# furio1999/EO_Diffusion

Hardware: AMD Instinct MI355X
Metric: denoising steps/sec (UNet fwd + DDPM update) at 256x256 bs=16 (higher is better)
Workload: dtype f32; 1 GPU; DDPM sampling step, 256x256x3, batch 16 per GPU, UNet arch A0 (base 128, mults [1,2,3,4], 1 res-block(s), attn_res []), Philox noise, x0-clipped update; global_batch=16, image_size=256, parallelism=batch-sharded x1, accumulate=fp32, precision_mode=fp32x3

## Files before the change

eo_diffusion_amd/_lib.py:

```python
import ctypes as C
import os

_HERE = os.path.dirname(os.path.abspath(__file__))
LIB_PATH = os.environ.get("EOD_LIBRARY") or os.path.join(_HERE, "lib", "libeodiff.so")

EOD_F32, EOD_F16 = 0, 1
ATTN_OUT_PRESPLIT, ATTN_IN_PRESPLIT, ATTN_EXACT_F32 = 1, 2, 4
(OP_CONV, OP_GEMM, OP_GN_PARTIAL, OP_GN_FINALIZE, OP_GN_APPLY, OP_SOFTMAX, OP_TEMB, OP_TO_NHWC, OP_TO_NCHW,
 OP_POOL, OP_ATTN, OP_TRANSPOSE, OP_ATTN_NAT, OP_DROPOUT, OP_ACT_BOUND, OP_BOUND_AFFINE) = range(1, 17)

vp, i32, i64, f32, f64 = C.c_void_p, C.c_int32, C.c_int64, C.c_float, C.c_double


class ConvDesc(C.Structure):
    _fields_ = [("x", vp), ("x2", vp), ("w", vp), ("bias", vp), ("cbias", vp), ("res", vp), ("y", vp),
                ("cbias_stride", i64), ("dtype", i32), ("N", i32), ("H", i32), ("W", i32), ("C0", i32), ("C1", i32),
                ("Cout", i32), ("ksize", i32), ("stride", i32), ("pad", i32), ("upsample", i32), ("pad_tl", i32),
                ("Ho", i32), ("Wo", i32), ("out_nchw_f32", i32), ("alpha", f32), ("stats", vp), ("stats_slots", i32),
                ("gn_silu", i32), ("gn_scale_shift", vp), ("workspace", vp), ("workspace_bytes", i64),
                ("w_tapmajor", i32), ("w_split", i32), ("w_scale", vp), ("a_bound", vp),
                ("skip_x", vp), ("skip_x2", vp), ("skip_w", vp), ("skip_C0", i32), ("skip_C1", i32), ("skip_bound", vp), ("x_presplit", i32), ("y_presplit_bound", vp)]


class GemmDesc(C.Structure):
# ... 67 lines not shown
    "eod_dropout": (i32, [vp, vp, i32, i64, f32, C.c_uint64, C.c_uint32, C.c_uint32, vp]),
    "eod_rowdot": (i32, [vp, vp, i32, i64, i64, i64, i64, i64, i64, i32, vp, vp]),
    "eod_scale_f32": (i32, [vp, i64, f32, vp]),
    "eod_attention_fwd_nat": (i32, [vp, vp, vp, i32, i32, i32, i32, i32, i32, i32, i32, i32, i32, vp, i32, vp]),
    "eod_weight_l1max": (i32, [vp, i32, i32, vp, vp, vp]),
    "eod_bound_affine": (i32, [vp, vp, vp, i32, vp]),
    "eod_attention_bwd": (i32, [vp, vp, vp, vp, vp, i32, i32, i32, i32, i32, i32, i32, i32, i32, i32, vp]),
    "eod_gemm_tn": (i32, [vp, i64, vp, i64, vp, i64, i32, i32, i32, i32, f32, i32, i32, i64, i64, i64, i64, i64, i64, vp]),
    "eod_softmax_bwd_rows": (i32, [vp, i64, vp, i64, vp, i32, i64, i32, vp]),
    "eod_linear_bwd_small": (i32, [vp, i64, vp, vp, vp, vp, vp, i32, i32, i32, i32, f32, vp, vp, vp, vp, vp]),
    "eod_temb_pre1": (i32, [vp, vp, vp, vp, i32, i32, i32, vp, vp]),
    "eod_embedding_bwd": (i32, [vp, vp, i32, i32, i32, f32, vp, vp]),
    "eod_mse_loss": (i32, [vp, vp, i64, vp, vp, vp, i32, vp]),
    "eod_adamw_step": (i32, [vp, vp, vp, vp, i64, f64, f64, f64, f64, f64, i32, vp]),
    "eod_adamw_step_guarded": (i32, [vp, vp, vp, vp, i64, f64, f64, f64, f64, f64, i32, vp, vp, i32, vp]),
    "eod_ema_update": (i32, [vp, vp, i64, f64, vp]),
    "eod_pack_rows": (i32, [vp, i64, vp, vp, i64, i32, i32, i32, vp]),
    "eod_nchw_to_nhwc": (i32, [vp, i32, vp, i32, vp, i32, i32, i32, i32, i32, vp]),
    "eod_nhwc_to_nchw": (i32, [vp, i32, vp, i32, i32, i32, i32, vp]),
    "eod_gn_partial": (i32, [vp, i32, i32, i32, i32, vp, i32, i32, i32, vp]),
    "eod_gn_finalize": (i32, [vp, i32, i32, vp, i32, i32, i32, i64, i32, f32, vp, vp, vp, i64, vp, vp, vp, vp]),
    "eod_act_bound": (i32, [vp, i32, i32, i64, vp, i32, i32, vp, i32, i32, vp, i32, vp]),
    "eod_conv_stats_slots": (i32, [C.POINTER(ConvDesc)]),
    "eod_conv_gn_fusable": (i32, [C.POINTER(ConvDesc)]),
    "eod_conv_split_ok": (i32, [C.POINTER(ConvDesc)]),
    "eod_conv_skip_ok": (i32, [C.POINTER(ConvDesc)]),
    "eod_conv_up4_ok": (i32, [C.POINTER(ConvDesc)]),
    "eod_conv_up4_weights": (i32, [vp, vp, i32, i32, vp]),
    "eod_conv_up4_bwd_ok": (i32, [C.POINTER(ConvDesc)]),
    "eod_pack_conv_weight_split": (i32, [vp, vp, vp, i32, i32, i32, i32, vp]),
    "eod_pack_conv_weight_split_pair": (i32, [vp, vp, vp, vp, vp, i32, i32, i32, i32, i32, vp]),
    "eod_conv_workspace_size": (i64, [C.POINTER(ConvDesc)]),
    "eod_conv_kernel_name": (C.c_char_p, [C.POINTER(ConvDesc)]),
    "eod_gn_apply": (i32, [vp, i32, i32, i32, i32, vp, i32, i32, i32, vp, vp, vp]),
    "eod_attention_fwd": (i32, [C.POINTER(AttnDesc), vp]),
    "eod_softmax_rows": (i32, [vp, i64, vp, i64, i32, i64, i32, vp]),
    "eod_time_embed": (i32, [C.POINTER(TembDesc), vp]),
    "eod_timestep_embedding": (i32, [vp, vp, vp, i32, i32, vp]),
    "eod_q_sample": (i32, [vp, vp, vp, vp, vp, vp, i32, i64, i32, vp]),
    "eod_repaint_mix": (i32, [vp, vp, vp, vp, vp, vp, vp, vp, i32, i32, i64, i32, vp]),
    "eod_ddpm_step": (i32, [vp, vp, vp, vp, vp, vp, vp, vp, vp, i32, i64, i32, i32, vp]),
    "eod_ddim_step": (i32, [vp, vp, vp, f32, f32, f32, f32, f32, vp, vp, i64, vp]),
    "eod_cfg_combine": (i32, [vp, vp, f32, vp, i64, vp]),
    "eod_dpmpp_step": (i32, [vp, vp, vp, f32, f32, f32, f32, f32, f32, i32, vp, vp, i64, vp]),
    "eod_ddim_step_obs": (i32, [vp, vp, vp, f32, f32, f32, f32, f32, vp, vp, f32, C.POINTER(i32), i32, i32, i32, i32, i32, i32, i32, vp, vp, vp]),
    "eod_dpmpp_step_obs": (i32, [vp, vp, vp, f32, f32, f32, f32, f32, f32, i32, vp, vp, f32, C.POINTER(i32), i32, i32, i32, i32, i32, i32, i32,
                                 vp, vp, vp]),
    "eod_block_mean": (i32, [vp, C.POINTER(i32), vp, i32, i32, i32, i32, vp]),
    "eod_obs_project": (i32, [vp, vp, vp, f32, C.POINTER(i32), i32, i32, i32, i32, i32, i32, i32, vp, vp]),
    "eod_ddim_step_spec": (i32, [vp, vp, vp, f32, f32, f32, f32, f32, vp, vp, f32, C.POINTER(f32), C.POINTER(f32), i32, i32, i32, i32, i32, i32,
                                 i32, i32, vp, vp, vp]),
    "eod_dpmpp_step_spec": (i32, [vp, vp, vp, f32, f32, f32, f32, f32, f32, i32, vp, vp, f32, C.POINTER(f32), C.POINTER(f32), i32, i32, i32, i32,
                                  i32, i32, i32, i32, vp, vp, vp]),
    "eod_spec_project": (i32, [vp, vp, vp, f32, C.POINTER(f32), C.POINTER(f32), i32, i32, i32, i32, i32, i32, i32, i32, vp, vp]),
    "eod_spec_apply": (i32, [vp, C.POINTER(f32), i32, i32, vp, i32, i32, i32, i32, vp]),
    "eod_psf_residual": (i32, [vp, vp, vp, f32, C.POINTER(f32), i32, i32, C.POINTER(i32), i32, i32, i32, i32, i32, i32, i32, i32, vp, vp]),
    "eod_psf_apply": (i32, [vp, C.POINTER(f32), i32, i32, C.POINTER(i32), i32, vp, i32, i32, i32, i32, vp]),
    "eod_psf_update": (i32, [vp, vp, f32, C.POINTER(f32), i32, i32, C.POINTER(i32), i32, i32, i32, i32, i32, vp, vp]),
    "eod_psf_residual_mix": (i32, [vp, vp, vp, f32, C.POINTER(f32), i32, i32, C.POINTER(f32), i32, i32, i32, i32, i32, i32, i32, vp, vp]),
    "eod_psf_apply_mix": (i32, [vp, C.POINTER(f32), i32, i32, C.POINTER(f32), i32, vp, i32, i32, i32, i32, vp]),
    "eod_psf_update_mix": (i32, [vp, vp, f32, C.POINTER(f32), i32, i32, C.POINTER(f32), i32, i32, i32, i32, i32, vp, vp]),
    "eod_psf_residual_xy": (i32, [vp, vp, vp, f32, C.POINTER(f32), i32, C.POINTER(f32), i32, i32, C.POINTER(i32), C.POINTER(f32), i32, i32, i32, i32, i32,
                                  i32, i32, i32, vp, vp]),
    "eod_psf_apply_xy": (i32, [vp, C.POINTER(f32), i32, C.POINTER(f32), i32, i32, C.POINTER(i32), C.POINTER(f32), i32, vp, i32, i32, i32, i32, vp]),
    "eod_psf_update_xy": (i32, [vp, vp, f32, C.POINTER(f32), i32, C.POINTER(f32), i32, i32, C.POINTER(i32), C.POINTER(f32), i32, i32, i32, i32, i32,
                                vp, vp]),
# ... 22 lines not shown
    "eod_scene_stack_tile_active": (i32, [vp, vp, i32, i32, i32, i32, i32, vp, vp, i32, i32, vp]),
    "eod_scene_stack_keep_known": (i32, [vp, vp, vp, i32, vp, vp, i32, i32, i32, i32, i32, i32, i32, vp, vp]),
    "eod_scene_stats": (i32, [vp, vp, vp, i32, i64, vp]),
    "eod_program_run": (i32, [C.POINTER(Op), i32, vp]),
    "eod_timer_create": (vp, [i32, i32]),
    "eod_timer_destroy": (None, [vp]),
    "eod_timer_read": (i32, [vp, C.POINTER(f32)]),
    "eod_timer_set_mask": (i32, [vp, vp, i32]),
    "eod_program_run_timed": (i32, [C.POINTER(Op), i32, vp, vp]),
    "eod_resample2x": (i32, [vp, i32, i32, i32, i32, i32, i32, i32, vp, vp]),
}

_lib = None


class EodError(RuntimeError):
    pass


ABI_VERSION = 115
SPEC_GRID_BLOCKS = 4096


def lib():
    global _lib
    if _lib is not None:
        return _lib
    if not os.path.exists(LIB_PATH):
        raise EodError(
            f"libeodiff.so not found at {LIB_PATH}. Build it first (python -c 'import __graft_entry__ as g; g.build()' "
            "or make -C eo_diffusion_amd/csrc). There is no fallback path.")
    import torch
    L = C.CDLL(LIB_PATH)
    for name, (res, args) in SYMBOLS.items():
        fn = getattr(L, name)
        fn.restype, fn.argtypes = res, args
    if L.eod_version() != ABI_VERSION and os.environ.get("EOD_ABI_ANY", "0") != "1":
        raise EodError(f"ABI mismatch: {LIB_PATH} was built for revision {L.eod_version()} of include/eodiff.h, this binding mirrors {ABI_VERSION}")
    for kind, st in ((1, ConvDesc), (2, GemmDesc), (3, TembDesc), (4, SmallDesc), (5, Op), (6, AttnDesc)):
        if L.eod_struct_size(kind) != C.sizeof(st):
            raise EodError(f"ABI mismatch: struct kind {kind}: C {L.eod_struct_size(kind)} vs ctypes {C.sizeof(st)}")
    _lib = L
    return L


def check(rc, what=""):
    if rc != 0:
        msg = lib().eod_last_error()
        raise EodError(f"{what} failed (rc={rc}): {msg.decode() if msg else ''}")


def dtype_id(torch_dtype):
    import torch
    if torch_dtype == torch.float16:
        return EOD_F16
    if torch_dtype == torch.float32:
        return EOD_F32
    raise EodError(f"unsupported storage dtype {torch_dtype}")


def ptr(t):
    return 0 if t is None else t.data_ptr()
```

eo_diffusion_amd/csrc/igemm.hip:

```cpp
#include <type_traits>

#include "common.h"

struct IgemmP {
    const char* a0;
    const char* a1;
    const char* b;
    const float* bias;
    const float* cbias;
    const char* res;
    char* y;
    long long cbias_stride;
    int N, H, W, C0, C1, Cin, Cout, KS, stride, pad, ups, pad_tl, Ho, Wo, HoWo, Heff, Weff;
    int tw_log2, th;
    int tiles_pw, tiles_pi;
    long long lda, ldb, ldc, sa0, sa1, sb0, sb1, sc0, sc1;
    int nb1, bias_mode, c_f32;
    long long M;
    int Ncols, K, taps, KT, tiles_m, tiles_n, out_nchw;
    int kc0, kc1;
    int tapmajor_log2;
    int ldk;
    const float* gn_ss;
    int gn_silu;
// ... 133 lines not shown
            g.ty0 = ty * p.th;
            g.tx0 = (t - ty * p.tiles_pw) << p.tw_log2;
        } else {
            const long long m0 = (long long)tile_m * BM;
            g.n_first = (int)(m0 / p.HWd);
            g.rem_first = (int)(m0 - (long long)g.n_first * p.HWd);
        }
    } else {
        const int z = blockIdx.y;
        const int b0 = z / p.nb1, b1 = z - b0 * p.nb1;
        g.offA = b0 * p.sa0 + b1 * p.sa1;
        g.offB = b0 * p.sb0 + b1 * p.sb1;
        g.offC = b0 * p.sc0 + b1 * p.sc1;
    }
    return g;
}

#ifdef EOD_STAMP
__device__ unsigned long long g_eod_stamp[65536][16];
#define EOD_STAMP_AT(k)                                                                    \
    do {                                                                                   \
        if (threadIdx.x == 0 && blockIdx.x < 65536) {                                      \
            g_eod_stamp[blockIdx.x][2 * (k)] = __builtin_amdgcn_s_memrealtime();           \
            g_eod_stamp[blockIdx.x][2 * (k) + 1] = __builtin_amdgcn_s_memtime();           \
        }                                                                                  \
    } while (0)
extern "C" int eod_debug_read_stamps(unsigned long long* host, int n) {
    return (int)hipMemcpyFromSymbol(host, HIP_SYMBOL(g_eod_stamp), (size_t)n * 16 * sizeof(unsigned long long), 0, hipMemcpyDeviceToHost);
}
#else
#define EOD_STAMP_AT(k) do { } while (0)
#endif
#ifdef EOD_TSTAMP
__device__ unsigned long long g_eod_tstamp[2048][40];
extern "C" int eod_debug_read_tstamps(unsigned long long* host, int n) {
    return (int)hipMemcpyFromSymbol(host, HIP_SYMBOL(g_eod_tstamp), (size_t)n * 40 * sizeof(unsigned long long), 0, hipMemcpyDeviceToHost);
}
#define EOD_TSTAMP_AT(idx)                                                                                      \
    do {                                                                                                        \
        if (GN && wave == 1 && cc == 1 && k == 0) {                                                             \
            const unsigned long long ts_ = __builtin_amdgcn_s_memtime();                                        \
            if (lane == 0) reinterpret_cast<unsigned long long*>(sA + ABUF + PR * 128)[idx] = ts_;              \
        }                                                                                                       \
    } while (0)
#else
#define EOD_TSTAMP_AT(idx) do { } while (0)
#endif
__device__ __forceinline__ void map_tile(const IgemmP& p, int& tile_m, int& tile_n) {
    const int nwg = gridDim.x, bid = blockIdx.x;
    const int xcd = bid & 7, q = nwg >> 3, r = nwg & 7;
    const int swz = (xcd < r ? xcd * (q + 1) : r * (q + 1) + (xcd - r) * q) + (bid >> 3);
    tile_n = swz % p.tiles_n;
    tile_m = swz / p.tiles_n;
}

template <int MS> struct AccLayout {
    static constexpr int R = MS == 32 ? 16 : 4;
    typedef typename std::conditional<MS == 32, f32x16, f32x4>::type vec;
    static __device__ __forceinline__ int row(int r, int lane) { return MS == 32 ? (r & 3) + 8 * (r >> 2) + 4 * (lane >> 5) : 4 * (lane >> 4) + r; }
    static __device__ __forceinline__ int col(int lane) { return MS == 32 ? (lane & 31) : (lane & 15); }
};

template <typename T, bool CONV, int BM, int BN, int WAVES_M, int WAVES_N, bool OUTF32, int MS = 32>
__device__ __forceinline__ void igemm_epilogue(const IgemmP& p, const TileGeom& g,
                                               typename AccLayout<MS>::vec (&acc)[BM / WAVES_M / MS][BN / WAVES_N / MS], char* smem, int wave,
                                               int lane, int n0, const float* rowtab = nullptr, int rowtab_n = 0,
                                               const float* pre_bcol = nullptr) {
    constexpr int ES = sizeof(T);
    constexpr int WM = BM / WAVES_M, WN = BN / WAVES_N;
    constexpr int TM = WM / MS, TN = WN / MS, R = AccLayout<MS>::R;
    constexpr int EP_LD = WN + 4;
    const int wm = wave / WAVES_N, wn = wave % WAVES_N;
    const int lr = AccLayout<MS>::col(lane);
// ... 712 lines not shown
    } else {
        if (CONV ? p.splitk > 1 : p.c_f32 != 0)
            igemm_epilogue<T, CONV, BM, BN, WAVES_M, WAVES_N, true, MS>(pe, g, acc, smem, wave, lane, n0);
        else
            igemm_epilogue<T, CONV, BM, BN, WAVES_M, WAVES_N, false, MS>(pe, g, acc, smem, wave, lane, n0);
    }
}

template <int TN, int MS>
__device__ __forceinline__ void prefetch_bcol(const IgemmP& p, int ncols, int col0, int lane, int n_first, float (&out)[TN]) {
    const int lr = AccLayout<MS>::col(lane);
#pragma unroll
    for (int j = 0; j < TN; ++j) {
        const int col = col0 + j * MS + lr;
        const bool ok = col < ncols;
        float v = (ok && p.bias && p.bias_mode == 1) ? p.bias[col] : 0.0f;
        if (ok && p.cbias) v += p.cbias[(long long)n_first * p.cbias_stride + col];
        out[j] = v;
    }
}

template <typename T, int BN, int WAVES_M, int WAVES_N, bool UPS, bool GN, bool SPLIT = false, int MS = 32, bool SKIP = false, bool KSPLIT = false>
__global__ __launch_bounds__(64 * WAVES_M * WAVES_N, WAVES_N == 4 ? 1 : 2) void conv3x3_halo_kernel(const IgemmP p) {
    static_assert(!KSPLIT || (!UPS && BN == 128), "K slices: the 128-column 4-wave instances");
    static_assert(!SKIP || (MS == 16 && !UPS && WAVES_M == 2), "fused skip conv: 16x16x32 instances of the 8x16 tile");
    static_assert(!SPLIT || (sizeof(T) == 4 && MS == 16), "the split-fp16 product is a mode of fp32 storage, on 16x16x32 MFMAs");
    static_assert(MS == 32 || SPLIT || sizeof(T) == 2, "the 16x16x32 shape exists for the fp16 products only");
    constexpr bool XF = GN || SPLIT;
    constexpr bool DIRECT = SPLIT && MS == 16 && BN >= 64;
    constexpr int NW = WAVES_M * WAVES_N;
    constexpr int BM = WAVES_N == 4 ? 64 * WAVES_M : 32 * NW, TH = BM / 16, TW = 16;
    constexpr int PH = UPS ? TH / 2 + 2 : TH + 2, PW = UPS ? TW / 2 + 2 : TW + 2, PR = PH * PW;
    constexpr int PG = (PR + 7) / 8;
    constexpr int LAH = (PG + NW - 1) / NW;
    constexpr int ES = sizeof(T), EPC = 16 / ES, BKB = 128, BK = BKB / ES;
    constexpr int WM = BM / WAVES_M, WN = BN / WAVES_N, TM = WM / MS, TN = WN / MS;
    constexpr int GB = BN / 8, LB = GB / NW;
    constexpr int ABUF = PG * 1024, BSTAGE = BN * BKB, BSTAGES = 2;
    static_assert(GB % NW == 0 && LAH <= 6, "layout");

    extern __shared__ __attribute__((aligned(16))) char smem[];
    char* const sA = smem;
    char* const sB = smem + 2 * ABUF;
    char* const sS = sB + BSTAGES * BSTAGE;
    EOD_STAMP_AT(0);

    const int tid = threadIdx.x, lane = tid & 63;
    const int wave = __builtin_amdgcn_readfirstlane(tid >> 6);
    const int wm = wave / WAVES_N, wn = wave % WAVES_N;
    int tile_m, tile_n;
    map_tile(p, tile_m, tile_n);
    const int n0 = p.n_base + tile_n * BN;
    const TileGeom g = make_geom<true, BM>(p, tile_m);
    float pre_bcol[DIRECT ? 1 : TN];
    f32x4 pre_bq[DIRECT ? TN : 1];
    int pre_we[DIRECT ? TN : 1];
    if constexpr (DIRECT) {
        prefetch_bcol4<TN>(p, p.Ncols, n0 + wn * WN, lane, g.n_first, pre_bq);
        prefetch_wexp4<TN>(p, p.Ncols, n0 + wn * WN, p.w_row0, lane, pre_we);
    } else {
        prefetch_bcol<TN, MS>(p, p.Ncols, n0 + wn * WN, lane, g.n_first, pre_bcol);
    }
    float wsc1 = 1.0f;
    if constexpr (SPLIT) wsc1 = p.w_scale[1];
    AbScale asc = {EOD_SPLIT_ASCALE, 1.0f};
    const float silu_k = p.gn_silu ? -1.44269504088896341f : 0.0f, silu_c = p.gn_silu ? 0.0f : -__builtin_inff();
    if constexpr (SPLIT) {
        if (p.a_bound) asc = ab_scale_of(ab_wave_bound(p.a_bound, g.n_first));
        if constexpr (SKIP) {
            if (p.skip_bound) {
                const AbScale k = ab_scale_of(ab_wave_bound(p.skip_bound, g.n_first));
                if (k.s < asc.s) asc = k;
            }
        }
    }

    const int srow = lane >> 3, sslot = lane & 7;
    unsigned ppix[LAH];
    const int bchunk0 = sslot ^ ((4 * wave + (srow >> 1)) & 7);
    unsigned pck = 0;
    unsigned pvalid = 0;
#pragma unroll
    for (int i = 0; i < LAH; ++i) {
        const int prow = (wave + NW * i) * 8 + srow;
        const int px = prow - (prow / PW) * PW;
        pck |= (unsigned)(sslot ^ ((px >> 1) & 7)) << (3 * i);
    }
    auto set_tile_pieces = [&](const TileGeom& tg) {
#pragma unroll
        for (int i = 0; i < LAH; ++i) {
            const int prow = (wave + NW * i) * 8 + srow;
            const int py = prow / PW, px = prow - py * PW;
            const int hi = (UPS ? tg.ty0 / 2 : tg.ty0) - 1 + py, wi = (UPS ? tg.tx0 / 2 : tg.tx0) - 1 + px;
            const bool ok = (wave + NW * i) < PG && prow < PR && (unsigned)hi < (unsigned)p.H && (unsigned)wi < (unsigned)p.W;
            if (ok) pvalid |= 1u << i;
            ppix[i] = (unsigned)(hi * p.W + wi);
        }
    };
    set_tile_pieces(g);
    auto pchunk_of = [&](int i) { return (int)((pck >> (3 * i)) & 7u); };
    unsigned b_v[LB];
#pragma unroll
    for (int i = 0; i < LB; ++i) {
        const int row = (wave + NW * i) * 8 + srow;
        b_v[i] = (n0 + row < p.Ncols) ? (unsigned)(row * p.Cin * ES) + bchunk0 * 16 : EOD_OOB;
    }
    const __amdgpu_buffer_rsrc_t rsA0 = make_rsrc(p.a0 + (long long)g.n_first * p.H * p.W * p.C0 * ES);
    const __amdgpu_buffer_rsrc_t rsA1 = make_rsrc(p.a1 ? p.a1 + (long long)g.n_first * p.H * p.W * p.C1 * ES : p.a0);
    const __amdgpu_buffer_rsrc_t rsB = make_rsrc(p.b + (long long)n0 * p.Cin * ES);
    const int tapstride = p.Cout * p.Cin * ES;
    __amdgpu_buffer_rsrc_t rsS = rsB;
    if constexpr (GN)
        rsS = __builtin_amdgcn_make_buffer_rsrc(const_cast<float*>(p.gn_ss) + (long long)g.n_first * p.Cin * 2, 0, p.Cin * 8, 0x00020000);

    struct Chunk {
        int src, kin, cw;
        unsigned bk;
        bool ktail;
    };
    auto chunk_of = [&](int cc) {
        Chunk c;
        c.src = cc >= p.kc0 ? 1 : 0;
        const int ci = c.src ? cc - p.kc0 : cc;
        c.kin = ci * BK;
        c.cw = c.src ? p.C1 : p.C0;
        c.bk = (unsigned)(((c.src ? p.C0 : 0) + c.kin) * ES);
        c.ktail = c.kin + BK > c.cw;
        return c;
    };
    auto issue_patch_piece = [&](int i, const Chunk& c, char* abuf) {
        const int pc = pchunk_of(i);
        unsigned v = ((pvalid >> i) & 1u) ? ppix[i] * (unsigned)(c.cw * ES) + pc * 16 : EOD_OOB;
        if (__builtin_expect(c.ktail, 0)) v = (c.kin + pc * EPC < c.cw) ? v : EOD_OOB;
        if (c.src)
            blds16(rsA1, v, (unsigned)(c.kin * ES), abuf + (wave + NW * i) * 1024);
        else
            blds16(rsA0, v, (unsigned)(c.kin * ES), abuf + (wave + NW * i) * 1024);
    };
    auto issue_ss = [&](const Chunk& c, char* ssbuf) {
        const unsigned v = lane < 32 ? (unsigned)(lane * 16 + ((c.src ? p.C0 : 0) + c.kin) * 8) : EOD_OOB;
        __builtin_amdgcn_raw_ptr_buffer_load_lds(rsS, (lds_void*)ssbuf, 16, v, 0, 0, 0);
    };
    struct XfPre {
        i32x4 raw;
        f32x4 q[GN ? (ES == 2 ? 4 : 2) : 1];
    };
    auto xf_load = [&](int i, char* abuf, const char* ssbuf, XfPre& pre) {
        const int pc = pchunk_of(i);
        pre.raw = *reinterpret_cast<const i32x4*>(abuf + (wave + NW * i) * 1024 + lane * 16);
        if constexpr (GN) {
            const float* sp = reinterpret_cast<const float*>(ssbuf) + pc * EPC * 2;
#pragma unroll
            for (int k = 0; k < (ES == 2 ? 4 : 2); ++k) pre.q[k] = *reinterpret_cast<const f32x4*>(sp + 4 * k);
        }
    };
    auto xf_finish = [&](int i, const Chunk& c, char* abuf, const XfPre& pre) {
        const int pc = pchunk_of(i);
        const bool ok = ((pvalid >> i) & 1u) && (!c.ktail || (c.kin + pc * EPC < c.cw));
        char* ptr = abuf + (wave + NW * i) * 1024 + lane * 16;
        const i32x4 raw = pre.raw;
        i32x4 outv = raw;
        if constexpr (GN) {
            if constexpr (ES == 2) {
                const half8 h = __builtin_bit_cast(half8, raw);
                half8 o;
#pragma unroll
                for (int e = 0; e < 8; ++e) {
                    float v = (float)h[e] * pre.q[e >> 1][(e & 1) * 2] + pre.q[e >> 1][(e & 1) * 2 + 1];
                    v = v * __builtin_amdgcn_rcpf(1.0f + __builtin_amdgcn_exp2f(__builtin_fmaf(v, silu_k, silu_c)));
                    o[e] = (half_t)v;
                }
                outv = __builtin_bit_cast(i32x4, o);
            } else {
                const f32x4 f = __builtin_bit_cast(f32x4, raw);
                f32x4 o;
                const f32x4 q0 = pre.q[0], q1 = pre.q[GN && ES != 2 ? 1 : 0];
                const float sc[4] = {q0[0], q0[2], q1[0], q1[2]}, sh[4] = {q0[1], q0[3], q1[1], q1[3]};
#pragma unroll
                for (int e = 0; e < 4; ++e) {
                    float v = f[e] * sc[e] + sh[e];
                    if constexpr (SPLIT) {
                        v = v * __builtin_amdgcn_rcpf(1.0f + __builtin_amdgcn_exp2f(__builtin_fmaf(v, silu_k, silu_c)));
                    } else {
                        if (p.gn_silu) v = silu_f<SPLIT>(v);
                    }
                    o[e] = v;
                }
                outv = __builtin_bit_cast(i32x4, o);
            }
            if constexpr (!SPLIT) {
                if (!ok) outv = raw;
            }
        }
        if constexpr (SPLIT) {
            const float sl = (GN && !ok) ? 0.0f : asc.s;
            *reinterpret_cast<i32x4*>(ptr) = split_pair_exchange_scaled(__builtin_bit_cast(f32x4, outv), sl, (pc & 1) != 0);
        } else {
            if (ok) *reinterpret_cast<i32x4*>(ptr) = outv;
        }
    };
    auto transform_piece = [&](int i, const Chunk& c, char* abuf, const char* ssbuf) {
        XfPre pre;
        xf_load(i, abuf, ssbuf, pre);
        xf_finish(i, c, abuf, pre);
    };
    unsigned bve[LB];
    auto weight_offsets = [&](const Chunk& c, unsigned (&out)[LB]) {
        const bool kok = !c.ktail || (c.kin + (SPLIT ? (bchunk0 >> 1) * 8 : bchunk0 * EPC) < c.cw);
#pragma unroll
        for (int i = 0; i < LB; ++i) out[i] = kok ? b_v[i] : EOD_OOB;
    };
    auto issue_weights_at = [&](int tap, const Chunk& c, const unsigned (&off)[LB], char* bst) {
        const unsigned soff = (unsigned)(tap * tapstride) + c.bk;
#pragma unroll
        for (int i = 0; i < LB; ++i) blds16(rsB, off[i], soff, bst + (wave + NW * i) * 1024);
    };
    auto issue_weights = [&](int tap, const Chunk& c, char* bst) {
        unsigned off[LB];
        weight_offsets(c, off);
        issue_weights_at(tap, c, off, bst);
    };

    typename AccLayout<MS>::vec acc[TM][TN];
#pragma unroll
    for (int i = 0; i < TM; ++i)
#pragma unroll
        for (int j = 0; j < TN; ++j)
#pragma unroll
            for (int r = 0; r < AccLayout<MS>::R; ++r) acc[i][j][r] = 0.0f;

    const int lr = lane & (MS - 1), lh = MS == 32 ? lane >> 5 : lane >> 4;
    int prow0[TM], pyo[TM], pxo[TM];
#pragma unroll
    for (int i = 0; i < TM; ++i) {
        const int r = wm * WM + i * MS + lr;
        pyo[i] = r >> 4;
        pxo[i] = r & 15;
        prow0[i] = pyo[i] * PW + pxo[i];
    }
    const int bsw = (lr >> 1) & 7;
    int bcoff[4];
#pragma unroll
    for (int s = 0; s < 4; ++s) bcoff[s] = ((2 * s + lh) ^ bsw) * 16;
    const int b_rd = (wn * WN + lr) * BKB;
    int acur[2][3] = {{0, 0, 0}, {0, 0, 0}};
    auto aoff = [](int r) { return (UPS ? ((r + 1) >> 1) : r) * PW * BKB; };
    i32x4 aw[2][TM];
    auto a_load = [&](int v, int dx, int dy) {
#pragma unroll
        for (int r = 0; r < TM + 2; ++r)
            if (dy == 0 ? r < TM : r == TM - 1 + dy) aw[v][r % TM] = *reinterpret_cast<const i32x4*>(sA + acur[v][dx] + aoff(r));
    };
    constexpr bool EARLY = MS == 16 && WAVES_N == 4;
    auto tap_slot = [](int t) { return MS == 16 ? 3 * (t % 3) + t / 3 : t; };
    if constexpr (MS == 16) {
        constexpr int LROW = WM / 16;
        static_assert(LROW % 2 == 0, "the UPS row split needs an even first tile row per wave");
        const int c0 = SPLIT ? 2 * ((0x2130 >> (4 * lh)) & 3) : lh, c1 = SPLIT ? c0 + 1 : 4 + lh;
#pragma unroll
        for (int dx = 0; dx < 3; ++dx) {
            const int pxc = UPS ? ((lr + dx + 1) >> 1) : lr + dx;
            const int key = (pxc >> 1) & 7;
            const int rowb = ((UPS ? (wm * LROW) >> 1 : wm * LROW) * PW + pxc) * BKB;
            acur[0][dx] = rowb + ((c0 ^ key) << 4);
            acur[1][dx] = rowb + ((c1 ^ key) << 4);
        }
    }

    const int KC = p.kc0 + p.kc1;
    int kc_begin = 0, kc_end = KC;
    if constexpr (KSPLIT) {
        kc_begin = (int)blockIdx.y * p.splitk_per;
        kc_end = (int)blockIdx.y == p.splitk - 1 ? KC : kc_begin + p.splitk_per;
    }
    const int NSTEP = (kc_end - kc_begin) * 9;
    {
        const Chunk c0 = chunk_of(kc_begin);
#pragma unroll
        for (int i = 0; i < LAH; ++i)
            if ((wave + NW * i) < PG) issue_patch_piece(i, c0, sA);
        if constexpr (GN) {
            if (wave == 0) issue_ss(c0, sS);
        }
        issue_weights(0, c0, sB);
        if constexpr (XF) {
            asm volatile("s_waitcnt vmcnt(0)" ::: "memory");
            if constexpr (GN) __builtin_amdgcn_s_barrier();
#pragma unroll
            for (int i = 0; i < LAH; ++i)
                if ((wave + NW * i) < PG) transform_piece(i, c0, sA, sS);
            __builtin_amdgcn_s_waitcnt(0xc07f);
        }
    }
    EOD_STAMP_AT(1);
    int pp1 = 0;
    int step = 0;
    int qpar = 0;
    for (int once = 0; once < 1; ++once) {
    for (int cc = kc_begin; cc < kc_end; ++cc) {
        const Chunk cur = chunk_of(cc);
        const int cn = cc + 1 < kc_end ? cc + 1 : cc;
        const bool has_next = cn != cc;
        const Chunk nxt = chunk_of(cn);
        const char* abuf = sA + qpar * ABUF;
        char* abuf_next = sA + (qpar ^ 1) * ABUF;
        weight_offsets(cur, bve);
#pragma unroll
        for (int t = 0; t < 9; ++t, ++step) {
            EOD_TSTAMP_AT(4 * t + 0);
            if (pp1 == 0) asm volatile("s_waitcnt vmcnt(0)" ::: "memory");
            else if (pp1 == 1) asm volatile("s_waitcnt vmcnt(1)" ::: "memory");
            else asm volatile("s_waitcnt vmcnt(2)" ::: "memory");
            if constexpr (XF) __builtin_amdgcn_s_waitcnt(0xc07f);
            __builtin_amdgcn_s_barrier();
            EOD_TSTAMP_AT(4 * t + 1);
            if (step + 1 < NSTEP) {
                if (t < 8) issue_weights_at(tap_slot(t + 1), cur, bve, sB + ((step + 1) & 1) * BSTAGE);
                else issue_weights(0, nxt, sB + ((step + 1) & 1) * BSTAGE);
            }
            pp1 = 0;
            if (t < LAH && has_next && (wave + NW * t) < PG) {
                issue_patch_piece(t, nxt, abuf_next);
                pp1 = 1;
            }
            if constexpr (GN) {
                if (t == 0 && has_next && wave == 0) {
                    issue_ss(nxt, sS + (qpar ^ 1) * 1024);
                    ++pp1;
                }
            }
            EOD_TSTAMP_AT(4 * t + 2);
            const int dy = MS == 16 ? t % 3 : t / 3, dx = MS == 16 ? t / 3 : t % 3;
            const int ndy = (t + 1) % 3, ndx = (t + 1) / 3;
            const bool a_here = !EARLY || t == 0, a_early = EARLY && t < 8;
            const char* bst = sB + (step & 1) * BSTAGE;
            int arow[TM], asw[TM];
#pragma unroll
            for (int i = 0; i < TM; ++i) {
                const int pxc = UPS ? ((pxo[i] + dx + 1) >> 1) : pxo[i] + dx;
                const int prow = UPS ? ((pyo[i] + dy + 1) >> 1) * PW + pxc : prow0[i] + dy * PW + dx;
                arow[i] = prow * BKB;
                asw[i] = (pxc >> 1) & 7;
            }
            if constexpr (MS == 16 && SPLIT) {
                const int ch = 2 * ((0x2130 >> (4 * lh)) & 3);
                i32x4 bh[TN], bl[TN];
                if (a_here) a_load(1, dx, dy);
#pragma unroll
                for (int j = 0; j < TN; ++j) bh[j] = *reinterpret_cast<const i32x4*>(bst + b_rd + j * MS * BKB + ((ch ^ bsw) << 4));
                if (a_here) a_load(0, dx, dy);
#pragma unroll
                for (int i = 0; i < TM; ++i)
#pragma unroll
                    for (int j = 0; j < TN; ++j)
                        acc[i][j] = DIRECT ? __builtin_amdgcn_mfma_f32_16x16x32_f16(__builtin_bit_cast(half8, bh[j]), __builtin_bit_cast(half8, aw[1][(i + dy) % TM]), acc[i][j], 0, 0, 0)
                                           : __builtin_amdgcn_mfma_f32_16x16x32_f16(__builtin_bit_cast(half8, aw[1][(i + dy) % TM]), __builtin_bit_cast(half8, bh[j]), acc[i][j], 0, 0, 0);
#pragma unroll
                for (int j = 0; j < TN; ++j) bl[j] = *reinterpret_cast<const i32x4*>(bst + b_rd + j * MS * BKB + (((ch + 1) ^ bsw) << 4));
                if (a_early) a_load(1, ndx, ndy);
#pragma unroll
                for (int i = 0; i < TM; ++i)
#pragma unroll
// ... 20 lines not shown
#pragma unroll
                        for (int j = 0; j < TN; ++j)
                            acc[i][j] = __builtin_amdgcn_mfma_f32_16x16x32_f16(__builtin_bit_cast(half8, aw[s][(i + dy) % TM]), __builtin_bit_cast(half8, fb16[j]), acc[i][j], 0, 0, 0);
                    if (a_early) a_load(s, ndx, ndy);
                }
            } else {
            i32x4 fa[2][TM], fb[2][TN];
#pragma unroll
            for (int i = 0; i < TM; ++i)
                fa[0][i] = *reinterpret_cast<const i32x4*>(abuf + arow[i] + (((0 + lh) ^ asw[i]) << 4));
#pragma unroll
            for (int j = 0; j < TN; ++j) fb[0][j] = *reinterpret_cast<const i32x4*>(bst + b_rd + j * 32 * BKB + bcoff[0]);
            __builtin_amdgcn_sched_group_barrier(0x100, TM + TN, 0);
#pragma unroll
            for (int s = 0; s < 4; ++s) {
                const int cur = s & 1, nx = cur ^ 1;
                if (s < 3) {
#pragma unroll
                    for (int i = 0; i < TM; ++i)
                        fa[nx][i] = *reinterpret_cast<const i32x4*>(abuf + arow[i] + (((2 * (s + 1) + lh) ^ asw[i]) << 4));
#pragma unroll
                    for (int j = 0; j < TN; ++j)
                        fb[nx][j] = *reinterpret_cast<const i32x4*>(bst + b_rd + j * 32 * BKB + bcoff[s + 1]);
                    __builtin_amdgcn_sched_group_barrier(0x100, TM + TN, 0);
                }
#pragma unroll
                for (int i = 0; i < TM; ++i)
#pragma unroll
                    for (int j = 0; j < TN; ++j) Mma<T>::run(fa[cur][i], fb[cur][j], acc[i][j]);
                __builtin_amdgcn_sched_group_barrier(0x008, TM * TN * (sizeof(T) == 4 ? 4 : 1), 0);
            }
            }
            EOD_TSTAMP_AT(4 * t + 3);
            if constexpr (XF) {
                if (t >= 2 && t - 2 < LAH && has_next && (wave + NW * (t - 2)) < PG)
                    transform_piece(t - 2, nxt, abuf_next, sS + (qpar ^ 1) * 1024);
            }
        }
        EOD_TSTAMP_AT(36);
#ifdef EOD_TSTAMP
        if (GN && wave == 1 && cc == 1 && blockIdx.x < 2048) {
            __builtin_amdgcn_s_waitcnt(0xc07f);
            if (lane < 37) g_eod_tstamp[blockIdx.x][lane] = reinterpret_cast<const unsigned long long*>(sA + ABUF + PR * 128)[lane];
        }
#endif
        if constexpr (MS == 16) {
            const int flip = qpar ? -ABUF : ABUF;
#pragma unroll
            for (int dx = 0; dx < 3; ++dx) {
                acur[0][dx] += flip;
                acur[1][dx] += flip;
            }
        }
        qpar ^= 1;
    }
    if constexpr (SKIP) {
      if (!KSPLIT || (int)blockIdx.y == p.splitk - 1) {
        constexpr int LA = BM / 8 / NW;
        constexpr int STG_A = BM * BKB, STG = STG_A + BSTAGE;
        static_assert(2 * STG <= 2 * ABUF + BSTAGES * BSTAGE, "the skip phase reuses the operand ring");
        __builtin_amdgcn_s_waitcnt(0xc07f);
        __builtin_amdgcn_s_barrier();
        const int SC = p.SC0 + p.SC1;
        const __amdgpu_buffer_rsrc_t rsX0 = make_rsrc(p.sx0 + (long long)g.n_first * p.H * p.W * p.SC0 * ES);
        const __amdgpu_buffer_rsrc_t rsX1 = make_rsrc(p.sx1 ? p.sx1 + (long long)g.n_first * p.H * p.W * p.SC1 * ES : p.sx0);
        const __amdgpu_buffer_rsrc_t rsW2 = make_rsrc(p.b2 + (long long)n0 * SC * ES);
        unsigned xpix[LA], wv[LB];
        unsigned xok = 0;
#pragma unroll
        for (int i = 0; i < LA; ++i) {
            const int row = (wave + NW * i) * 8 + srow;
            xpix[i] = (unsigned)((g.ty0 + (row >> 4)) * p.W + g.tx0 + (row & 15));
            if (g.tx0 + (row & 15) < p.W) xok |= 1u << i;
        }
// ... 1458 lines not shown
        } else if (on256 && d->Cout % 256 == 0 && d->N * tiles_pi * (d->Cout / 256) >= 256 && ((gn && !exact) || (split && skip))) {
            pl.bn = 256;
        } else if (on256 && d->Cout > 256 && d->Cout % 256 == 128 && d->N * tiles_pi * ((d->Cout - 128) / 256) >= 256 && split && gn) {
            pl.bn = 256;
            pl.plus128 = true;
        }
    } else {
        pl.family = pl.splitk <= 1 && !split && conv_parity_ok(d, Ho, Wo) ? FAM_GENERIC_PARITY : FAM_GENERIC;
        pl.bn = generic_bn(d->Cout);
        if (split && d->Cout > 64) {
            const long long M = (long long)d->N * Ho * Wo;
            if (d->Cout % 256 == 0 && pl.splitk <= 1 && ((M + 127) / 128) * (d->Cout / 256) >= 256 && opt(OPT_HALO_BN256)) pl.bn = 256;
            pl.direct = pl.splitk <= 1 && !d->out_nchw_f32 && (Ho * Wo) % 128 == 0 && M % 128 == 0 && d->Cout % 4 == 0;
        }
    }
    return pl;
}

extern "C" int eod_conv_skip_ok(const eod_conv_desc* d) { return d && conv_plan(d).skip_ok ? 1 : 0; }
extern "C" int eod_conv_gn_fusable(const eod_conv_desc* d) { return d && conv_plan(d).gn_fusable ? 1 : 0; }
extern "C" int64_t eod_conv_workspace_size(const eod_conv_desc* d) { return d ? conv_plan(d).workspace_bytes : 0; }
extern "C" int eod_conv_stats_slots(const eod_conv_desc* d) { return d ? conv_plan(d).stats_slots : 0; }
extern "C" const char* eod_conv_kernel_name(const eod_conv_desc* d) {
    if (!d) return "";
    const ConvPlan pl = conv_plan(d);
    switch (pl.family) {
        case FAM_UP4: case FAM_UP4_BWD: return "conv_up4_halo_kernel";
        case FAM_FIRST: return "conv_first_x3_kernel";
        case FAM_S2_HALO: return "conv_s2_halo_kernel";
        case FAM_HEAD: return "conv_head_kernel";
        case FAM_HALO: return pl.bn == 32 ? "conv3x3_halo_kernel<BN=32>" : "conv3x3_halo_kernel";
        default: return "igemm_kernel";
    }
}

static int conv_up4_bwd(const eod_conv_desc* d, void* stream) {
    EOD_REQUIRE(d->N > 0 && d->H > 0 && d->W > 0 && d->C0 > 0 && d->Cout > 0 && d->x && d->w && d->y, "conv (upsample 4): bad args");
    EOD_REQUIRE(conv_up4_bwd_ok(d), "conv: upsample = 4 needs a geometry for which eod_conv_up4_bwd_ok(d) == 1");
    EOD_REQUIRE(eod_aligned16(d->x) && eod_aligned16(d->w), "conv: 16-byte alignment");
    EOD_REQUIRE((long long)d->H * d->W * d->C0 * 2 < 0x7fffffffLL && 9LL * d->Cout * 4 * d->C0 * 2 < 0x7fffffffLL, "conv (upsample 4): operand exceeds the 2 GiB window");
    const ConvPlan pl = conv_plan(d);
    IgemmP p = {};
    p.a0 = (const char*)d->x; p.b = (const char*)d->w; p.bias = d->bias; p.bias_mode = d->bias ? 1 : 0;
    p.cbias = d->cbias; p.cbias_stride = d->cbias_stride; p.res = (const char*)d->res; p.y = (char*)d->y;
    p.N = d->N; p.H = pl.Ho; p.W = pl.Wo;
    p.C0 = d->C0; p.C1 = 0; p.Cin = d->C0; p.Cout = d->Cout; p.KS = 3; p.stride = 1; p.pad = 1;
    p.Ho = pl.Ho; p.Wo = pl.Wo; p.HoWo = pl.Ho * pl.Wo; p.Heff = pl.Heff; p.Weff = pl.Weff;
    p.Hd = pl.Ho; p.Wd = pl.Wo; p.HWd = pl.Ho * pl.Wo;
    p.M = (long long)d->N * pl.Ho * pl.Wo; p.Ncols = d->Cout; p.taps = 9; p.alpha = d->alpha; p.nb1 = 1; p.tapmajor_log2 = -1;
    return launch_up4<half_t, false, true>(p, (hipStream_t)stream);
}

static IgemmP splitk_partial(const IgemmP& p, const eod_conv_desc* d, const ConvPlan& pl) {
    IgemmP q = p;
    q.stats = nullptr;
    q.splitk = pl.splitk;
    q.splitk_per = pl.splitk_per;
    q.y = (char*)d->workspace;
    q.bias = nullptr; q.bias_mode = 0; q.cbias = nullptr; q.res = nullptr; q.alpha = 1.0f;
    return q;
}
static int splitk_finish(const eod_conv_desc* d, const IgemmP& p, int splitk, hipStream_t st) {
    if (d->stats) {
        const dim3 grid((unsigned)((p.Cout + 63) / 64), (unsigned)d->N);
        if (d->dtype == EOD_F16)
            hipLaunchKernelGGL(splitk_reduce_stats_kernel<half_t>, grid, dim3(256), 0, st, (const float*)d->workspace, splitk, p.M, p.Cout, p.HoWo, d->alpha, d->bias, d->cbias, (long long)d->cbias_stride, (const half_t*)d->res, (half_t*)d->y, d->stats);
// ... 238 lines not shown
```

include/eodiff.h:

```cpp
#ifndef EODIFF_H
#define EODIFF_H

#include <stdint.h>

#ifdef __cplusplus
extern "C" {
#endif

#define EOD_OK 0
#define EOD_EINVAL (-1)
#define EOD_ELAUNCH (-2)
#define EOD_ENOSYS (-3)

enum { EOD_F32 = 0, EOD_F16 = 1 };

const char* eod_last_error(void);
#define EOD_ABI_VERSION 115
int eod_version(void);
int eod_set_option(const char* name, int value);
int eod_get_option(const char* name);
int eod_struct_size(int kind);

typedef struct {
    const void* x;
// ... 13 lines not shown
    int32_t upsample;
    int32_t pad_tl;
    int32_t Ho, Wo;
    int32_t out_nchw_f32;
    float alpha;
    float* stats;
    int32_t stats_slots;
    int32_t gn_silu;
    const float* gn_scale_shift;
    void* workspace;
    int64_t workspace_bytes;
    int32_t w_tapmajor;
    int32_t w_split;
    const float* w_scale;
    const float* a_bound;
    const void* skip_x;
    const void* skip_x2;
    const void* skip_w;
    int32_t skip_C0, skip_C1;
    const float* skip_bound;
    int32_t x_presplit;
    const float* y_presplit_bound;
} eod_conv_desc;
int eod_conv2d_igemm(const eod_conv_desc* d, void* stream);
int eod_conv_stats_slots(const eod_conv_desc* d);
int eod_conv_gn_fusable(const eod_conv_desc* d);
int eod_conv_split_ok(const eod_conv_desc* d);
int eod_conv_skip_ok(const eod_conv_desc* d);
int eod_conv_up4_ok(const eod_conv_desc* d);
int eod_conv_up4_weights(const float* w_oihw, float* wc, int Cout, int Cin, void* stream);
int eod_conv_up4_bwd_ok(const eod_conv_desc* d);
int64_t eod_conv_workspace_size(const eod_conv_desc* d);
const char* eod_conv_kernel_name(const eod_conv_desc* d);

typedef struct {
    const void* a;
    const void* b;
    const float* bias;
    const void* res;
    void* c;
    int64_t lda, ldb, ldc;
    int64_t sa0, sa1, sb0, sb1, sc0, sc1;
    int32_t dtype;
    int32_t M, N, K;
    int32_t nb0, nb1;
    int32_t bias_mode;
    int32_t c_f32;
    float alpha;
    int32_t x3;
    const float* a_bound;
    const float* b_bound;
} eod_gemm_desc;
int eod_gemm_nt(const eod_gemm_desc* d, void* stream);

int eod_pack_conv_weight(const float* w_oihw, void* dst, int dtype, int Cout, int Cin, int ksize,
                         int cin_pad, void* stream);
int eod_pack_conv_weight_split(const float* w_oihw, void* dst, float* scale, int Cout, int Cin, int ksize, int cin_pad, void* stream);
int eod_pack_conv_weight_split_pair(const float* w_oihw, void* dst, const float* w2_oi, void* dst2, float* scale, int Cout, int Cin,
                                    int ksize, int cin_pad, int Cin2, void* stream);
int eod_pack_conv_weight_tapmajor(const float* w_oihw, void* dst, int dtype, int Cout, int Cin, int cin_pad, void* stream);
int eod_pack_conv_weight_tapmajor_split(const float* w_oihw, void* dst, float* scale, int Cout, int Cin, int cin_pad, void* stream);
int eod_conv_tapmajor_ldk(int C0, int dtype);
int eod_pack_rows(const float* src, int64_t ld_src, const int32_t* row_map, void* dst, int64_t ld_dst,
                  int dtype, int rows, int cols, void* stream);

int eod_nchw_to_nhwc(const float* src0, int C0, const float* src1, int C1, void* dst, int dtype,
// ... 253 lines not shown
```

Before: 40.74 steps/s.

## Split halo conv waves into weight-loader and patch-loader roles

In the 3x3 halo conv kernel, when WAVES_N==4 and MS==16, the waves are split by wm into two roles. wm==1 waves issue all the next-step weight tiles, and wm==0 waves issue and transform the next chunk's activation patch pieces, each with its own vmcnt waits. The goal is to cut the per-step global-load wait that stalls every wave and to overlap the loads better with MFMA work. In exchange the waves become asymmetric, and a new static_assert restricts this path to XF configurations with even piece counts. The change also adds a query for the halo column count, makes the timestamp wave configurable, and tolerates missing symbols under EOD_ABI_ANY.

```diff
diff --git a/eo_diffusion_amd/_lib.py b/eo_diffusion_amd/_lib.py
--- a/eo_diffusion_amd/_lib.py
+++ b/eo_diffusion_amd/_lib.py
@@ -123,6 +123,7 @@
     "eod_pack_conv_weight_split_pair": (i32, [vp, vp, vp, vp, vp, i32, i32, i32, i32, i32, vp]),
     "eod_conv_workspace_size": (i64, [C.POINTER(ConvDesc)]),
     "eod_conv_kernel_name": (C.c_char_p, [C.POINTER(ConvDesc)]),
+    "eod_conv_halo_columns": (i32, [C.POINTER(ConvDesc)]),
     "eod_gn_apply": (i32, [vp, i32, i32, i32, i32, vp, i32, i32, i32, vp, vp, vp]),
     "eod_attention_fwd": (i32, [C.POINTER(AttnDesc), vp]),
     "eod_softmax_rows": (i32, [vp, i64, vp, i64, i32, i64, i32, vp]),
@@ -211,7 +212,10 @@
             "or make -C eo_diffusion_amd/csrc). There is no fallback path.")
     import torch
     L = C.CDLL(LIB_PATH)
+    abi_any = os.environ.get("EOD_ABI_ANY", "0") == "1"
     for name, (res, args) in SYMBOLS.items():
+        if abi_any and not hasattr(L, name):
+            continue
         fn = getattr(L, name)
         fn.restype, fn.argtypes = res, args
     if L.eod_version() != ABI_VERSION and os.environ.get("EOD_ABI_ANY", "0") != "1":
diff --git a/eo_diffusion_amd/csrc/igemm.hip b/eo_diffusion_amd/csrc/igemm.hip
--- a/eo_diffusion_amd/csrc/igemm.hip
+++ b/eo_diffusion_amd/csrc/igemm.hip
@@ -189,13 +189,16 @@
 #define EOD_STAMP_AT(k) do { } while (0)
 #endif
 #ifdef EOD_TSTAMP
+#ifndef EOD_TSTAMP_WAVE
+#define EOD_TSTAMP_WAVE 1
+#endif
 __device__ unsigned long long g_eod_tstamp[2048][40];
 extern "C" int eod_debug_read_tstamps(unsigned long long* host, int n) {
     return (int)hipMemcpyFromSymbol(host, HIP_SYMBOL(g_eod_tstamp), (size_t)n * 40 * sizeof(unsigned long long), 0, hipMemcpyDeviceToHost);
 }
 #define EOD_TSTAMP_AT(idx)                                                                                      \
     do {                                                                                                        \
-        if (GN && wave == 1 && cc == 1 && k == 0) {                                                             \
+        if (GN && wave == EOD_TSTAMP_WAVE && cc == 1) {                                                         \
             const unsigned long long ts_ = __builtin_amdgcn_s_memtime();                                        \
             if (lane == 0) reinterpret_cast<unsigned long long*>(sA + ABUF + PR * 128)[idx] = ts_;              \
         }                                                                                                       \
@@ -974,12 +977,16 @@
     constexpr int BM = WAVES_N == 4 ? 64 * WAVES_M : 32 * NW, TH = BM / 16, TW = 16;
     constexpr int PH = UPS ? TH / 2 + 2 : TH + 2, PW = UPS ? TW / 2 + 2 : TW + 2, PR = PH * PW;
     constexpr int PG = (PR + 7) / 8;
-    constexpr int LAH = (PG + NW - 1) / NW;
+    constexpr bool ROLES = WAVES_N == 4 && MS == 16;
+    constexpr int RW = ROLES ? 4 : NW;
+    constexpr int LAH = (PG + RW - 1) / RW;
     constexpr int ES = sizeof(T), EPC = 16 / ES, BKB = 128, BK = BKB / ES;
     constexpr int WM = BM / WAVES_M, WN = BN / WAVES_N, TM = WM / MS, TN = WN / MS;
-    constexpr int GB = BN / 8, LB = GB / NW;
+    constexpr int GB = BN / 8, LB = GB / NW, LBR = GB / RW;
+    constexpr int LBV = ROLES ? 1 : LB;
     constexpr int ABUF = PG * 1024, BSTAGE = BN * BKB, BSTAGES = 2;
     static_assert(GB % NW == 0 && LAH <= 6, "layout");
+    static_assert(!ROLES || (XF && GB % RW == 0 && LAH % 2 == 0 && LBR % 2 == 0), "role split: in-place rewrite; the prologue halves the pieces");
 
     extern __shared__ __attribute__((aligned(16))) char smem[];
     char* const sA = smem;
@@ -990,6 +997,7 @@
     const int tid = threadIdx.x, lane = tid & 63;
     const int wave = __builtin_amdgcn_readfirstlane(tid >> 6);
     const int wm = wave / WAVES_N, wn = wave % WAVES_N;
+    const int wr = ROLES ? wn : wave;
     int tile_m, tile_n;
     map_tile(p, tile_m, tile_n);
     const int n0 = p.n_base + tile_n * BN;
@@ -1024,28 +1032,29 @@
     unsigned pvalid = 0;
 #pragma unroll
     for (int i = 0; i < LAH; ++i) {
-        const int prow = (wave + NW * i) * 8 + srow;
+        const int prow = (wr + RW * i) * 8 + srow;
         const int px = prow - (prow / PW) * PW;
         pck |= (unsigned)(sslot ^ ((px >> 1) & 7)) << (3 * i);
     }
     auto set_tile_pieces = [&](const TileGeom& tg) {
 #pragma unroll
         for (int i = 0; i < LAH; ++i) {
-            const int prow = (wave + NW * i) * 8 + srow;
+            const int prow = (wr + RW * i) * 8 + srow;
             const int py = prow / PW, px = prow - py * PW;
             const int hi = (UPS ? tg.ty0 / 2 : tg.ty0) - 1 + py, wi = (UPS ? tg.tx0 / 2 : tg.tx0) - 1 + px;
-            const bool ok = (wave + NW * i) < PG && prow < PR && (unsigned)hi < (unsigned)p.H && (unsigned)wi < (unsigned)p.W;
+            const bool ok = (wr + RW * i) < PG && prow < PR && (unsigned)hi < (unsigned)p.H && (unsigned)wi < (unsigned)p.W;
             if (ok) pvalid |= 1u << i;
             ppix[i] = (unsigned)(hi * p.W + wi);
         }
     };
     set_tile_pieces(g);
     auto pchunk_of = [&](int i) { return (int)((pck >> (3 * i)) & 7u); };
-    unsigned b_v[LB];
-#pragma unroll
-    for (int i = 0; i < LB; ++i) {
-        const int row = (wave + NW * i) * 8 + srow;
-        b_v[i] = (n0 + row < p.Ncols) ? (unsigned)(row * p.Cin * ES) + bchunk0 * 16 : EOD_OOB;
+    unsigned b_v[LBV];
+    const int brem = ROLES ? p.Ncols - n0 - (wr * 8 + srow) : 0;
+#pragma unroll
+    for (int i = 0; i < LBV; ++i) {
+        const int row = (wr + RW * i) * 8 + srow;
+        b_v[i] = (ROLES || n0 + row < p.Ncols) ? (unsigned)(row * p.Cin * ES) + bchunk0 * 16 : EOD_OOB;
     }
     const __amdgpu_buffer_rsrc_t rsA0 = make_rsrc(p.a0 + (long long)g.n_first * p.H * p.W * p.C0 * ES);
     const __amdgpu_buffer_rsrc_t rsA1 = make_rsrc(p.a1 ? p.a1 + (long long)g.n_first * p.H * p.W * p.C1 * ES : p.a0);
@@ -1075,9 +1084,9 @@
         unsigned v = ((pvalid >> i) & 1u) ? ppix[i] * (unsigned)(c.cw * ES) + pc * 16 : EOD_OOB;
         if (__builtin_expect(c.ktail, 0)) v = (c.kin + pc * EPC < c.cw) ? v : EOD_OOB;
         if (c.src)
-            blds16(rsA1, v, (unsigned)(c.kin * ES), abuf + (wave + NW * i) * 1024);
+            blds16(rsA1, v, (unsigned)(c.kin * ES), abuf + (wr + RW * i) * 1024);
         else
-            blds16(rsA0, v, (unsigned)(c.kin * ES), abuf + (wave + NW * i) * 1024);
+            blds16(rsA0, v, (unsigned)(c.kin * ES), abuf + (wr + RW * i) * 1024);
     };
     auto issue_ss = [&](const Chunk& c, char* ssbuf) {
         const unsigned v = lane < 32 ? (unsigned)(lane * 16 + ((c.src ? p.C0 : 0) + c.kin) * 8) : EOD_OOB;
@@ -1089,7 +1098,7 @@
     };
     auto xf_load = [&](int i, char* abuf, const char* ssbuf, XfPre& pre) {
         const int pc = pchunk_of(i);
-        pre.raw = *reinterpret_cast<const i32x4*>(abuf + (wave + NW * i) * 1024 + lane * 16);
+        pre.raw = *reinterpret_cast<const i32x4*>(abuf + (wr + RW * i) * 1024 + lane * 16);
         if constexpr (GN) {
             const float* sp = reinterpret_cast<const float*>(ssbuf) + pc * EPC * 2;
 #pragma unroll
@@ -1099,7 +1108,7 @@
     auto xf_finish = [&](int i, const Chunk& c, char* abuf, const XfPre& pre) {
         const int pc = pchunk_of(i);
         const bool ok = ((pvalid >> i) & 1u) && (!c.ktail || (c.kin + pc * EPC < c.cw));
-        char* ptr = abuf + (wave + NW * i) * 1024 + lane * 16;
+        char* ptr = abuf + (wr + RW * i) * 1024 + lane * 16;
         const i32x4 raw = pre.raw;
         i32x4 outv = raw;
         if constexpr (GN) {
@@ -1146,21 +1155,27 @@
         xf_load(i, abuf, ssbuf, pre);
         xf_finish(i, c, abuf, pre);
     };
-    unsigned bve[LB];
-    auto weight_offsets = [&](const Chunk& c, unsigned (&out)[LB]) {
+    unsigned bve[LBV];
+    auto weight_offsets = [&](const Chunk& c, unsigned (&out)[LBV]) {
         const bool kok = !c.ktail || (c.kin + (SPLIT ? (bchunk0 >> 1) * 8 : bchunk0 * EPC) < c.cw);
 #pragma unroll
-        for (int i = 0; i < LB; ++i) out[i] = kok ? b_v[i] : EOD_OOB;
-    };
-    auto issue_weights_at = [&](int tap, const Chunk& c, const unsigned (&off)[LB], char* bst) {
+        for (int i = 0; i < LBV; ++i) out[i] = kok ? b_v[i] : EOD_OOB;
+    };
+    auto issue_weights_at = [&](int tap, const Chunk& c, const unsigned (&off)[LBV], char* bst) {
         const unsigned soff = (unsigned)(tap * tapstride) + c.bk;
 #pragma unroll
-        for (int i = 0; i < LB; ++i) blds16(rsB, off[i], soff, bst + (wave + NW * i) * 1024);
+        for (int i = 0; i < LBV; ++i) blds16(rsB, off[i], soff, bst + (wr + RW * i) * 1024);
     };
     auto issue_weights = [&](int tap, const Chunk& c, char* bst) {
-        unsigned off[LB];
+        unsigned off[LBV];
         weight_offsets(c, off);
         issue_weights_at(tap, c, off, bst);
+    };
+    auto issue_weight_tile = [&](int tap, const Chunk& c, unsigned off, char* bst, int i0, int i1) {
+        const unsigned soff = (unsigned)(tap * tapstride) + c.bk;
+#pragma unroll
+        for (int i = 0; i < LBR; ++i)
+            if (i >= i0 && i < i1) blds16(rsB, brem > RW * 8 * i ? off : EOD_OOB, soff + (unsigned)(RW * 8 * i * p.Cin * ES), bst + (wr + RW * i) * 1024);
     };
 
     typename AccLayout<MS>::vec acc[TM][TN];
@@ -1218,9 +1233,25 @@
     const int NSTEP = (kc_end - kc_begin) * 9;
     {
         const Chunk c0 = chunk_of(kc_begin);
+        if constexpr (ROLES) {
+#pragma unroll
+            for (int i = 0; i < LAH; ++i)
+                if ((i >= LAH / 2) == (wm != 0) && (wr + RW * i) < PG) issue_patch_piece(i, c0, sA);
+            if constexpr (GN) {
+                if (wave == 0) issue_ss(c0, sS);
+            }
+            weight_offsets(c0, bve);
+            issue_weight_tile(0, c0, bve[0], sB, wm * (LBR / 2), (wm + 1) * (LBR / 2));
+            asm volatile("s_waitcnt vmcnt(0)" ::: "memory");
+            if constexpr (GN) __builtin_amdgcn_s_barrier();
+#pragma unroll
+            for (int i = 0; i < LAH; ++i)
+                if ((i >= LAH / 2) == (wm != 0) && (wr + RW * i) < PG) transform_piece(i, c0, sA, sS);
+            __builtin_amdgcn_s_waitcnt(0xc07f);
+        } else {
 #pragma unroll
         for (int i = 0; i < LAH; ++i)
-            if ((wave + NW * i) < PG) issue_patch_piece(i, c0, sA);
+            if ((wr + RW * i) < PG) issue_patch_piece(i, c0, sA);
         if constexpr (GN) {
             if (wave == 0) issue_ss(c0, sS);
         }
@@ -1230,8 +1261,9 @@
             if constexpr (GN) __builtin_amdgcn_s_barrier();
 #pragma unroll
             for (int i = 0; i < LAH; ++i)
-                if ((wave + NW * i) < PG) transform_piece(i, c0, sA, sS);
+                if ((wr + RW * i) < PG) transform_piece(i, c0, sA, sS);
             __builtin_amdgcn_s_waitcnt(0xc07f);
+        }
         }
     }
     EOD_STAMP_AT(1);
@@ -1250,18 +1282,34 @@
 #pragma unroll
         for (int t = 0; t < 9; ++t, ++step) {
             EOD_TSTAMP_AT(4 * t + 0);
-            if (pp1 == 0) asm volatile("s_waitcnt vmcnt(0)" ::: "memory");
-            else if (pp1 == 1) asm volatile("s_waitcnt vmcnt(1)" ::: "memory");
-            else asm volatile("s_waitcnt vmcnt(2)" ::: "memory");
+            if constexpr (ROLES) {
+                if (wm == 1) asm volatile("s_waitcnt vmcnt(0)" ::: "memory");
+                else if (GN && t == 2) asm volatile("s_waitcnt vmcnt(2)" ::: "memory");
+            } else {
+                if (pp1 == 0) asm volatile("s_waitcnt vmcnt(0)" ::: "memory");
+                else if (pp1 == 1) asm volatile("s_waitcnt vmcnt(1)" ::: "memory");
+                else asm volatile("s_waitcnt vmcnt(2)" ::: "memory");
+            }
             if constexpr (XF) __builtin_amdgcn_s_waitcnt(0xc07f);
             __builtin_amdgcn_s_barrier();
             EOD_TSTAMP_AT(4 * t + 1);
+            if constexpr (ROLES) {
+                if (wm == 1 && step + 1 < NSTEP) {
+                    if (t < 8) {
+                        issue_weight_tile(tap_slot(t + 1), cur, bve[0], sB + ((step + 1) & 1) * BSTAGE, 0, LBR);
+                    } else {
+                        unsigned off[LBV];
+                        weight_offsets(nxt, off);
+                        issue_weight_tile(0, nxt, off[0], sB + ((step + 1) & 1) * BSTAGE, 0, LBR);
+                    }
+                }
+            } else {
             if (step + 1 < NSTEP) {
                 if (t < 8) issue_weights_at(tap_slot(t + 1), cur, bve, sB + ((step + 1) & 1) * BSTAGE);
                 else issue_weights(0, nxt, sB + ((step + 1) & 1) * BSTAGE);
             }
             pp1 = 0;
-            if (t < LAH && has_next && (wave + NW * t) < PG) {
+            if (t < LAH && has_next && (wr + RW * t) < PG) {
                 issue_patch_piece(t, nxt, abuf_next);
                 pp1 = 1;
             }
@@ -1270,6 +1318,7 @@
                     issue_ss(nxt, sS + (qpar ^ 1) * 1024);
                     ++pp1;
                 }
+            }
             }
             EOD_TSTAMP_AT(4 * t + 2);
             const int dy = MS == 16 ? t % 3 : t / 3, dx = MS == 16 ? t / 3 : t % 3;
@@ -1356,14 +1405,32 @@
             }
             }
             EOD_TSTAMP_AT(4 * t + 3);
-            if constexpr (XF) {
-                if (t >= 2 && t - 2 < LAH && has_next && (wave + NW * (t - 2)) < PG)
+            if constexpr (ROLES) {
+                if (wm == 0 && has_next) {
+                    int now = 0;
+                    if constexpr (GN) {
+                        if (t == 0 && wave == 0) issue_ss(nxt, sS + (qpar ^ 1) * 1024);
+                    }
+                    if (t < LAH && (wr + RW * t) < PG) {
+                        issue_patch_piece(t, nxt, abuf_next);
+                        now = 1;
+                    }
+                    if (t >= 2 && t - 2 < LAH && (wr + RW * (t - 2)) < PG) {
+                        if (pp1 + now == 0) asm volatile("s_waitcnt vmcnt(0)" ::: "memory");
+                        else if (pp1 + now == 1) asm volatile("s_waitcnt vmcnt(1)" ::: "memory");
+                        else asm volatile("s_waitcnt vmcnt(2)" ::: "memory");
+                        transform_piece(t - 2, nxt, abuf_next, sS + (qpar ^ 1) * 1024);
+                    }
+                    pp1 = now;
+                }
+            } else if constexpr (XF) {
+                if (t >= 2 && t - 2 < LAH && has_next && (wr + RW * (t - 2)) < PG)
                     transform_piece(t - 2, nxt, abuf_next, sS + (qpar ^ 1) * 1024);
             }
         }
         EOD_TSTAMP_AT(36);
 #ifdef EOD_TSTAMP
-        if (GN && wave == 1 && cc == 1 && blockIdx.x < 2048) {
+        if (GN && wave == EOD_TSTAMP_WAVE && cc == 1 && blockIdx.x < 2048) {
             __builtin_amdgcn_s_waitcnt(0xc07f);
             if (lane < 37) g_eod_tstamp[blockIdx.x][lane] = reinterpret_cast<const unsigned long long*>(sA + ABUF + PR * 128)[lane];
         }
@@ -2888,6 +2955,12 @@
         case FAM_HALO: return pl.bn == 32 ? "conv3x3_halo_kernel<BN=32>" : "conv3x3_halo_kernel";
         default: return "igemm_kernel";
     }
+}
+
+extern "C" int eod_conv_halo_columns(const eod_conv_desc* d) {
+    if (!d) return 0;
+    const ConvPlan pl = conv_plan(d);
+    return pl.family == FAM_HALO ? pl.bn : 0;
 }
 
 static int conv_up4_bwd(const eod_conv_desc* d, void* stream) {
diff --git a/include/eodiff.h b/include/eodiff.h
--- a/include/eodiff.h
+++ b/include/eodiff.h
@@ -69,6 +69,7 @@
 int eod_conv_up4_bwd_ok(const eod_conv_desc* d);
 int64_t eod_conv_workspace_size(const eod_conv_desc* d);
 const char* eod_conv_kernel_name(const eod_conv_desc* d);
+int eod_conv_halo_columns(const eod_conv_desc* d);
 
 typedef struct {
     const void* a;
```

Result: faster. 41.24 steps/s (median of 6 runs) (+1.2%).
